# k2-fsa/Flow2GAN

Measured on AMD Instinct MI355X. Metric: audio-seconds/sec (train step, G+D fwd/bwd) mel_24k_base, higher is better.
Workload: dtype f32 (fp32-class products on the bf16 matrix pipe for the long reductions and the direct MRD convs: every fp32 operand as three bf16 pieces = 24 significand bits, the six v_mfma_f32_32x32x16_bf16 products with i + j <= 2 per fp32 product, fp32 accumulate, error <= 2^-23 per product; short reductions ; 1 GPU; mel_24k_base GAN stage-2 train step: D-step + G-step, each on its own batch (MPD+MRD+FM+multi-scale mel), fwd+bwd+grad all-reduce, no optimizer (metric is fwd/bwd); per_gpu_batch=64, gan=gan_multi_scale_mel_recon, parallelism=dp1, optimizer=none

## Files before the change

flow2gan_amd/csrc/conv32x6.hip:

```cpp
#include <stdlib.h>

#include "common.h"


namespace {

typedef float f32x16 __attribute__((ext_vector_type(16)));
typedef float f32x4 __attribute__((ext_vector_type(4)));
typedef __bf16 bf16x8 __attribute__((ext_vector_type(8)));
typedef unsigned int u32x2 __attribute__((ext_vector_type(2)));
typedef unsigned int u32x4 __attribute__((ext_vector_type(4)));

constexpr int C = 32, KH = 3, KW = 9, NTAP = KH * KW;
constexpr int PB = 208;
constexpr int TG = 4;
constexpr int WBB = C * PB;
constexpr int WCH = C * 12;

__device__ __attribute__((aligned(16))) float c6_zero[4] = {0.f, 0.f, 0.f, 0.f};

__device__ __forceinline__ void split3(const f32x4 v, u32x2& p0, u32x2& p1, u32x2& p2) {
  unsigned a0, a1, a2, b0, b1, b2;
  f2g_split3_pair(v.x, v.y, a0, a1, a2);
  f2g_split3_pair(v.z, v.w, b0, b1, b2);
  p0 = u32x2{a0, b0};
  p1 = u32x2{a1, b1};
  p2 = u32x2{a2, b2};
}

__device__ __forceinline__ void store_px3(unsigned char* p, const f32x4 v) {
  u32x2 p0, p1, p2;
  split3(v, p0, p1, p2);
// ... 31 lines not shown
  return (x * (D == 39 ? 1681 : D == 23 ? 2850 : D == 20 ? 3277 : 5462)) >> 16;
}

template <int TW_>
__device__ __forceinline__ void px_of_row(int pg, int r, int& ph, int& pw) {
  if (TW_ == 16) {
    ph = 2 * pg + (r >> 4);
    pw = (r + 12 * (r >> 4)) & 15;
  } else {
    const int p = pg * 32 + r;
    ph = p / TW_;
    pw = p % TW_;
  }
}

struct wplan {
  int src[3];
  int dst[3];
  int u[3];
};

template <int TH_, int TW_>
__global__ __launch_bounds__(512, 1) void conv32_s2_fwd6_kernel(const f2g_conv32_desc d, int tiles_w,
                                                               int tiles_h, int ntiles) {
  constexpr int IHv = TH_ + KH - 1, IWv = TW_ + (KW - 1) / 2, XW = 2 * IWv - 1;
  constexpr int SUBB = IHv * IWv * PB + 64;
  constexpr int NCHK = (IHv * XW * (C / 4) + 511) / 512;
  constexpr int NG = (NTAP + TG - 1) / TG + 1;
  static_assert(NG % 2 == 0, "the weight double buffer must come back to buffer 0 at a tile's end");
  static_assert(TH_ * TW_ == 128, "a block owns 128 output pixels");
  extern __shared__ __attribute__((aligned(16))) unsigned char smb[];
  unsigned char* At = smb;
  unsigned char* Bt = smb + 2 * SUBB;
  float* red = reinterpret_cast<float*>(Bt + 2 * TG * WBB);
  const int tid = threadIdx.x, lane = tid & 63, wave = tid >> 6;
  const int li = lane & 31, hh = lane >> 5;
  const int pg = wave & 3, half = wave >> 2;
  const int c4 = tid & 7;
  const int px0 = tid >> 3;
  auto tile_pos = [&](int tile, int& sq, int& h0, int& w0) {
    const int tw = tile % tiles_w, rest = tile / tiles_w;
    const int th = rest % tiles_h;
    sq = rest / tiles_h;
    h0 = th * TH_;
    w0 = tw * TW_;
  };
  auto load_patch = [&](int tile, f32x4 (&pf)[NCHK]) {
    int sq, h0, w0;
    tile_pos(tile, sq, h0, w0);
    const int x0 = 2 * w0 - (KW - 1) / 2;
    const float* org = d.x + (long long)sq * d.x_seq + (long long)(h0 - 1) * d.x_line + (long long)x0 * C + c4 * 4;
#pragma unroll
    for (int q = 0; q < NCHK; ++q) {
      const int px = px0 + 64 * q;
      const int r = div_small<XW>(px), xr = px - r * XW;
      const int h = h0 - 1 + r, x = x0 + xr;
      const bool ok = px < IHv * XW && h >= 0 && h < d.H && x >= 0 && x < d.Win;
      pf[q] = *reinterpret_cast<const f32x4*>(ok ? org + (long long)r * d.x_line + xr * C : c6_zero);
    }
  };
  auto store_patch = [&](const f32x4 (&pf)[NCHK]) {
#pragma unroll
    for (int q = 0; q < NCHK; ++q) {
      const int px = px0 + 64 * q;
      const int r = div_small<XW>(px), xr = px - r * XW;
      if (px < IHv * XW) store_px3(At + (xr & 1) * SUBB + (r * IWv + (xr >> 1)) * PB + c4 * 8, pf[q]);
    }
  };
  const unsigned char* wimg = reinterpret_cast<const unsigned char*>(d.w);
  wplan wp;
#pragma unroll
  for (int k = 0; k < 3; ++k) {
    const int c = tid + 512 * k;
    const int u = c / WCH, rem = c - u * WCH;
    const int row = rem / 12, part = rem - row * 12;
    wp.u[k] = u;
    wp.src[k] = row * (NTAP * 192) + part * 16;
    wp.dst[k] = u * WBB + row * PB + part * 16;
  }
  auto load_w = [&](int g, u32x4 (&wn)[3]) {
#pragma unroll
    for (int k = 0; k < 3; ++k) {
      int t = g * TG + wp.u[k];
      t = t < NTAP ? t : NTAP - 1;
      wn[k] = *reinterpret_cast<const u32x4*>(wimg + wp.src[k] + t * 192);
    }
  };
  auto store_w = [&](int buf, const u32x4 (&wn)[3]) {
#pragma unroll
    for (int k = 0; k < 3; ++k) *reinterpret_cast<u32x4*>(Bt + buf * (TG * WBB) + wp.dst[k]) = wn[k];
  };
  int ph, pw;
  px_of_row<TW_>(pg, li, ph, pw);
  const unsigned char* Ap = At + (ph * IWv + pw) * PB + hh * 16;
  const unsigned char* Bp = Bt + li * PB + hh * 16;
  const float bias = d.bias ? d.bias[li] : 0.f;

  int tile = blockIdx.x;
  if (tile >= ntiles) return;
  u32x4 wn[3];
  {
    f32x4 pf[NCHK];
    load_patch(tile, pf);
    load_w(0, wn);
    store_patch(pf);
    store_w(0, wn);
  }
  __syncthreads();
#define F2G_C6_AOFF(T) ((((T) % KW) & 1) * SUBB + (((T) / KW) * IWv + (((T) % KW) >> 1)) * PB)
  for (; tile < ntiles; tile += gridDim.x) {
    const int nxt = tile + gridDim.x;
    const bool more = nxt < ntiles;
    f32x4 pf[NCHK];
    load_patch(more ? nxt : tile, pf);
    f32x16 acc0, acc1;
#pragma unroll
    for (int e = 0; e < 16; ++e) { acc0[e] = 0.f; acc1[e] = 0.f; }
#pragma unroll
    for (int g = 0; g < NG; ++g) {
      load_w(g + 1 < NG ? g + 1 : 0, wn);
      const int buf = g & 1;
#pragma unroll
      for (int u2 = 0; u2 < 2; ++u2) {
        const int t0 = g * TG + u2, t1 = g * TG + 2 + u2;
        if (t0 < NTAP && (half ? t1 : t0) < NTAP)
          tap6(Ap + (half ? F2G_C6_AOFF(t1) : F2G_C6_AOFF(t0)), Bp + (buf * TG + half * 2 + u2) * WBB, acc0, acc1);
      }
      store_w(buf ^ 1, wn);
      __syncthreads();
    }
#undef F2G_C6_AOFF
#pragma unroll
    for (int e = 0; e < 16; ++e) acc0[e] += acc1[e];
    if (half == 1) {
#pragma unroll
      for (int e = 0; e < 16; ++e) red[(pg * 16 + e) * 64 + lane] = acc0[e];
    }
    if (more) store_patch(pf);
    __syncthreads();
    if (half == 0) {
      int sq, h0, w0;
      tile_pos(tile, sq, h0, w0);
      float* ys = d.y + (long long)sq * d.y_seq;
      float* turn = red + pg * (16 * 64);
      float v[16];
#pragma unroll
      for (int e = 0; e < 16; ++e) {
        v[e] = acc0[e] + red[(pg * 16 + e) * 64 + lane] + bias;
        if (d.lrelu_slope != 0.f) v[e] = v[e] > 0.f ? v[e] : d.lrelu_slope * v[e];
      }
      __builtin_amdgcn_wave_barrier();
#pragma unroll
      for (int e = 0; e < 16; ++e) turn[((e & 3) + 8 * (e >> 2) + 4 * hh) * 32 + li] = v[e];
      __builtin_amdgcn_wave_barrier();
#pragma unroll
      for (int j = 0; j < 4; ++j) {
        int qh, qw;
        px_of_row<TW_>(pg, (lane >> 3) + 8 * j, qh, qw);
        const int oh = h0 + qh, ow = w0 + qw;
        const f32x4 u = *reinterpret_cast<const f32x4*>(turn + ((lane >> 3) + 8 * j) * 32 + 4 * (lane & 7));
        if (oh < d.H && ow < d.Wout)
          *reinterpret_cast<f32x4*>(ys + (long long)oh * d.y_line + (long long)ow * C + 4 * (lane & 7)) = u;
      }
    }
  }
}

template <int TH_, int TW_>
__global__ __launch_bounds__(512, 1) void conv32_s2_dgrad6_kernel(const f2g_conv32_desc d, int tiles_w,
                                                                 int tiles_h, int ntiles) {
  constexpr int IHv = TH_ + KH - 1, GWv = TW_ + 4;
  constexpr int NCHK = (IHv * GWv * (C / 4) + 511) / 512;
  constexpr int NG = 8;
  static_assert(TH_ * TW_ == 128, "a block owns 128 positions of each column parity");
  extern __shared__ __attribute__((aligned(16))) unsigned char smb[];
  unsigned char* At = smb;
  unsigned char* Bt = smb + IHv * GWv * PB;
  float* turn = reinterpret_cast<float*>(Bt + 2 * TG * WBB) + (threadIdx.x >> 6) * (32 * 32);
  const int tid = threadIdx.x, lane = tid & 63, wave = tid >> 6;
  const int li = lane & 31, hh = lane >> 5;
  const int pg = wave & 3, E = wave >> 2;
  const int c4 = tid & 7;
  const int NU = E ? 4 : 5, NT = KH * NU;
  const int Wp = (d.Win + 1 - E) / 2;
  const int px0 = tid >> 3;
  auto tile_pos = [&](int tile, int& sq, int& h0, int& m0) {
    const int tw = tile % tiles_w, rest = tile / tiles_w;
    const int th = rest % tiles_h;
    sq = rest / tiles_h;
    h0 = th * TH_;
    m0 = tw * TW_;
  };
  auto load_patch = [&](int tile, f32x4 (&pf)[NCHK]) {
    int sq, h0, m0;
    tile_pos(tile, sq, h0, m0);
    const float* org = d.x + (long long)sq * d.x_seq + (long long)(h0 - 1) * d.x_line + (long long)(m0 - 2) * C + c4 * 4;
#pragma unroll
    for (int q = 0; q < NCHK; ++q) {
      const int px = px0 + 64 * q;
      const int r = div_small<GWv>(px), xc = px - r * GWv;
      const int h = h0 - 1 + r, c = m0 - 2 + xc;
      const bool ok = px < IHv * GWv && h >= 0 && h < d.H && c >= 0 && c < d.Wout;
      pf[q] = *reinterpret_cast<const f32x4*>(ok ? org + (long long)r * d.x_line + xc * C : c6_zero);
    }
  };
  auto store_patch = [&](const f32x4 (&pf)[NCHK]) {
#pragma unroll
    for (int q = 0; q < NCHK; ++q) {
      const int px = px0 + 64 * q;
      if (px < IHv * GWv) store_px3(At + px * PB + c4 * 8, pf[q]);
    }
  };
  const unsigned char* wimg = reinterpret_cast<const unsigned char*>(d.w);
  int wsrc[3], wdst[3], wslot[3];
#pragma unroll
  for (int k = 0; k < 3; ++k) {
    const int c = tid + 512 * k;
    const int u = c / WCH, rem = c - u * WCH;
    const int row = rem / 12, part = rem - row * 12;
    wslot[k] = u;
    wsrc[k] = row * 192 + part * 16;
    wdst[k] = u * WBB + row * PB + part * 16;
  }
  auto load_w = [&](int g, u32x4 (&wn)[3]) {
#pragma unroll
    for (int k = 0; k < 3; ++k) {
      const int e = wslot[k] >> 1, nu = e ? 4 : 5, nt = KH * nu;
      int ti = 2 * g + (wslot[k] & 1);
      ti = ti < nt ? ti : nt - 1;
      const int dh = e ? ti >> 2 : (ti * 13) >> 6;
      const int tile_w = dh * KW + e + 2 * (ti - dh * nu);
      wn[k] = *reinterpret_cast<const u32x4*>(wimg + (long long)tile_w * (C * 192) + wsrc[k]);
    }
  };
  auto store_w = [&](int buf, const u32x4 (&wn)[3]) {
#pragma unroll
    for (int k = 0; k < 3; ++k) *reinterpret_cast<u32x4*>(Bt + buf * (TG * WBB) + wdst[k]) = wn[k];
  };
  int ph, pw;
  px_of_row<TW_>(pg, li, ph, pw);
  const unsigned char* Ap = At + ((ph + 2) * GWv + pw + 4) * PB + hh * 16;
  const unsigned char* Bp = Bt + (E * 2) * WBB + li * PB + hh * 16;
  const bool msk = d.mask_src != nullptr, fm = d.fm_ref != nullptr;
  const float fmw = fm ? d.fm_w * (d.fm_wdev ? d.fm_wdev[0] : 1.f) : 0.f;
  float cs[4] = {0.f, 0.f, 0.f, 0.f};

  int tile = blockIdx.x;
  if (tile >= ntiles) return;
  u32x4 wn[3];
  {
    f32x4 pf[NCHK];
    load_patch(tile, pf);
    load_w(0, wn);
    store_patch(pf);
    store_w(0, wn);
  }
  __syncthreads();
  for (; tile < ntiles; tile += gridDim.x) {
    const int nxt = tile + gridDim.x;
    const bool more = nxt < ntiles;
    f32x4 pf[NCHK];
    load_patch(more ? nxt : tile, pf);
    int sq, h0, m0;
    tile_pos(tile, sq, h0, m0);
    long long ioff[4];
    f32x4 my[4];
#pragma unroll
    for (int j = 0; j < 4; ++j) {
      int qh, qw;
      px_of_row<TW_>(pg, (lane >> 3) + 8 * j, qh, qw);
      const int oh = h0 + qh, om = m0 + qw;
      ioff[j] = (oh < d.H && om < Wp)
                    ? (long long)sq * d.y_seq + (long long)oh * d.y_line + (long long)(2 * om + E) * C + 4 * (lane & 7)
                    : -1;
      if (msk && !fm) my[j] = *reinterpret_cast<const f32x4*>(d.mask_src + (ioff[j] >= 0 ? ioff[j] : 0));
    }
    f32x16 acc0, acc1;
#pragma unroll
    for (int e = 0; e < 16; ++e) { acc0[e] = 0.f; acc1[e] = 0.f; }
#define F2G_C6_GOFF(TI) ((E ? ((TI) / 4) * GWv + (TI) % 4 : ((TI) / 5) * GWv + (TI) % 5) * PB)
#pragma unroll
    for (int g = 0; g < NG; ++g) {
      load_w(g + 1 < NG ? g + 1 : 0, wn);
      const int buf = g & 1;
#pragma unroll
      for (int u2 = 0; u2 < 2; ++u2)
        if (2 * g + u2 < NT) tap6(Ap - F2G_C6_GOFF(2 * g + u2), Bp + (buf * TG + u2) * WBB, acc0, acc1);
      store_w(buf ^ 1, wn);
      __syncthreads();
    }
#undef F2G_C6_GOFF
#pragma unroll
    for (int q = 0; q < 16; ++q) turn[((q & 3) + 8 * (q >> 2) + 4 * hh) * 32 + li] = acc0[q] + acc1[q];
    __builtin_amdgcn_wave_barrier();
    auto item = [&](int j) {
      return *reinterpret_cast<const f32x4*>(turn + ((lane >> 3) + 8 * j) * 32 + 4 * (lane & 7));
    };
    if (!msk) {
#pragma unroll
      for (int j = 0; j < 4; ++j) {
        const f32x4 u = item(j);
        if (ioff[j] < 0) continue;
        cs[0] += u.x, cs[1] += u.y, cs[2] += u.z, cs[3] += u.w;
        *reinterpret_cast<f32x4*>(d.y + ioff[j]) = u;
      }
    } else if (!fm) {
#pragma unroll
      for (int j = 0; j < 4; ++j) {
        const f32x4 u = item(j);
        if (ioff[j] < 0) continue;
        f32x4 v;
        v.x = u.x * (my[j].x > 0.f ? 1.f : d.mask_slope);
        v.y = u.y * (my[j].y > 0.f ? 1.f : d.mask_slope);
        v.z = u.z * (my[j].z > 0.f ? 1.f : d.mask_slope);
        v.w = u.w * (my[j].w > 0.f ? 1.f : d.mask_slope);
        cs[0] += v.x, cs[1] += v.y, cs[2] += v.z, cs[3] += v.w;
        *reinterpret_cast<f32x4*>(d.y + ioff[j]) = v;
      }
    } else {
      f32x4 yv[4], fv[4];
#pragma unroll
      for (int j = 0; j < 4; ++j) {
        const long long o = ioff[j] >= 0 ? ioff[j] : 0;
        yv[j] = *reinterpret_cast<const f32x4*>(d.mask_src + o);
        fv[j] = *reinterpret_cast<const f32x4*>(d.fm_ref + o);
      }
#pragma unroll
      for (int j = 0; j < 4; ++j) {
        const f32x4 u = item(j);
        if (ioff[j] < 0) continue;
        float v[4] = {u.x, u.y, u.z, u.w};
        const float y[4] = {yv[j].x, yv[j].y, yv[j].z, yv[j].w}, f[4] = {fv[j].x, fv[j].y, fv[j].z, fv[j].w};
#pragma unroll
        for (int e = 0; e < 4; ++e) {
          const float dl = y[e] - f[e];
          v[e] += fmw * (dl > 0.f ? 1.f : (dl < 0.f ? -1.f : 0.f));
          v[e] *= y[e] > 0.f ? 1.f : d.mask_slope;
          cs[e] += v[e];
        }
        *reinterpret_cast<f32x4*>(d.y + ioff[j]) = f32x4{v[0], v[1], v[2], v[3]};
      }
    }
    __builtin_amdgcn_wave_barrier();
    if (more) store_patch(pf);
    __syncthreads();
  }
  if (d.colsum) {
#pragma unroll
    for (int e = 0; e < 4; ++e) {
      float v = cs[e];
      v += __shfl_xor(v, 8);
      v += __shfl_xor(v, 16);
      v += __shfl_xor(v, 32);
      if (lane < 8) atomicAdd(d.colsum + 4 * lane + e, v);
    }
  }
}

template <int TH_, int TW_>
__global__ __launch_bounds__(512, 1) void conv32_s2_dgrad6m_kernel(const f2g_conv32_desc d, int tiles_w,
                                                                 int tiles_h, int ntiles) {
  constexpr int IHv = TH_ + KH - 1, GWv = TW_ + 4;
  constexpr int NCHK = (IHv * GWv * (C / 4) + 511) / 512;
  constexpr int NG = 8;
  static_assert(TH_ * TW_ == 128, "a block owns 128 positions of each column parity");
  extern __shared__ __attribute__((aligned(16))) unsigned char smb[];
  unsigned char* At = smb;
  unsigned char* Bt = smb + IHv * GWv * PB;
  const int tid = threadIdx.x, lane = tid & 63, wave = tid >> 6;
  const int li = lane & 31, hh = lane >> 5;
  const int pg = wave & 3, E = wave >> 2;
  const int c4 = tid & 7;
  const int NU = E ? 4 : 5, NT = KH * NU;
  const int Wp = (d.Win + 1 - E) / 2;
  const int px0 = tid >> 3;
  auto tile_pos = [&](int tile, int& sq, int& h0, int& m0) {
    const int tw = tile % tiles_w, rest = tile / tiles_w;
    const int th = rest % tiles_h;
    sq = rest / tiles_h;
    h0 = th * TH_;
    m0 = tw * TW_;
  };
  auto load_patch = [&](int tile, f32x4 (&pf)[NCHK]) {
    int sq, h0, m0;
    tile_pos(tile, sq, h0, m0);
    const float* org = d.x + (long long)sq * d.x_seq + (long long)(h0 - 1) * d.x_line + (long long)(m0 - 2) * C + c4 * 4;
#pragma unroll
    for (int q = 0; q < NCHK; ++q) {
      const int px = px0 + 64 * q;
      const int r = div_small<GWv>(px), xc = px - r * GWv;
      const int h = h0 - 1 + r, c = m0 - 2 + xc;
      const bool ok = px < IHv * GWv && h >= 0 && h < d.H && c >= 0 && c < d.Wout;
      pf[q] = *reinterpret_cast<const f32x4*>(ok ? org + (long long)r * d.x_line + xc * C : c6_zero);
    }
  };
  auto store_patch = [&](const f32x4 (&pf)[NCHK]) {
#pragma unroll
    for (int q = 0; q < NCHK; ++q) {
      const int px = px0 + 64 * q;
      if (px < IHv * GWv) store_px3(At + px * PB + c4 * 8, pf[q]);
    }
  };
  const unsigned char* wimg = reinterpret_cast<const unsigned char*>(d.w);
  int wsrc[3], wdst[3], wslot[3];
#pragma unroll
  for (int k = 0; k < 3; ++k) {
    const int c = tid + 512 * k;
    const int u = c / WCH, rem = c - u * WCH;
    const int row = rem / 12, part = rem - row * 12;
    wslot[k] = u;
    wsrc[k] = row * 192 + part * 16;
    wdst[k] = u * WBB + row * PB + part * 16;
  }
  auto load_w = [&](int g, u32x4 (&wn)[3]) {
#pragma unroll
    for (int k = 0; k < 3; ++k) {
      const int e = wslot[k] >> 1, nu = e ? 4 : 5, nt = KH * nu;
      int ti = 2 * g + (wslot[k] & 1);
      ti = ti < nt ? ti : nt - 1;
      const int dh = e ? ti >> 2 : (ti * 13) >> 6;
      const int tile_w = dh * KW + e + 2 * (ti - dh * nu);
      wn[k] = *reinterpret_cast<const u32x4*>(wimg + (long long)tile_w * (C * 192) + wsrc[k]);
    }
  };
  auto store_w = [&](int buf, const u32x4 (&wn)[3]) {
#pragma unroll
    for (int k = 0; k < 3; ++k) *reinterpret_cast<u32x4*>(Bt + buf * (TG * WBB) + wdst[k]) = wn[k];
  };
  int ph, pw;
  px_of_row<TW_>(pg, li, ph, pw);
  const unsigned char* Ap = At + ((ph + 2) * GWv + pw + 4) * PB + hh * 16;
  const unsigned char* Bp = Bt + (E * 2) * WBB + li * PB + hh * 16;
  const bool msk = d.mask_src != nullptr, fm = d.fm_ref != nullptr;
  const float fmw = fm ? d.fm_w * (d.fm_wdev ? d.fm_wdev[0] : 1.f) : 0.f;
  float cs = 0.f;

  int tile = blockIdx.x;
  if (tile >= ntiles) return;
  u32x4 wn[3];
  {
    f32x4 pf[NCHK];
    load_patch(tile, pf);
    load_w(0, wn);
    store_patch(pf);
    store_w(0, wn);
  }
  __syncthreads();
  for (; tile < ntiles; tile += gridDim.x) {
    const int nxt = tile + gridDim.x;
    const bool more = nxt < ntiles;
    f32x4 pf[NCHK];
    load_patch(more ? nxt : tile, pf);
    int sq, h0, m0;
    tile_pos(tile, sq, h0, m0);
    float my[16];
    if (msk && !fm) {
#pragma unroll
      for (int q = 0; q < 16; ++q) {
        int qh, qw;
        px_of_row<TW_>(pg, (q & 3) + 8 * (q >> 2) + 4 * hh, qh, qw);
        const int oh = h0 + qh, om = m0 + qw;
        const long long off = (long long)sq * d.y_seq + (long long)oh * d.y_line + (long long)(2 * om + E) * C + li;
        my[q] = (oh < d.H && om < Wp) ? d.mask_src[off] : 1.f;
      }
    }
    f32x16 acc0, acc1;
#pragma unroll
    for (int e = 0; e < 16; ++e) { acc0[e] = 0.f; acc1[e] = 0.f; }
#define F2G_C6_GOFF(TI) ((E ? ((TI) / 4) * GWv + (TI) % 4 : ((TI) / 5) * GWv + (TI) % 5) * PB)
#pragma unroll
    for (int g = 0; g < NG; ++g) {
      load_w(g + 1 < NG ? g + 1 : 0, wn);
      const int buf = g & 1;
#pragma unroll
      for (int u2 = 0; u2 < 2; ++u2)
        if (2 * g + u2 < NT) tap6(Ap - F2G_C6_GOFF(2 * g + u2), Bp + (buf * TG + u2) * WBB, acc0, acc1);
      store_w(buf ^ 1, wn);
      __syncthreads();
    }
#undef F2G_C6_GOFF
#pragma unroll
    for (int q = 0; q < 16; ++q) {
      int qh, qw;
      px_of_row<TW_>(pg, (q & 3) + 8 * (q >> 2) + 4 * hh, qh, qw);
      const int oh = h0 + qh, om = m0 + qw;
      if (oh < d.H && om < Wp) {
        const long long off = (long long)sq * d.y_seq + (long long)oh * d.y_line + (long long)(2 * om + E) * C + li;
        float v = acc0[q] + acc1[q];
        if (msk) {
          const float y = fm ? d.mask_src[off] : my[q];
          if (fm) {
            const float dl = y - d.fm_ref[off];
            v += fmw * (dl > 0.f ? 1.f : (dl < 0.f ? -1.f : 0.f));
          }
          v *= y > 0.f ? 1.f : d.mask_slope;
        }
        cs += v;
        d.y[off] = v;
      }
    }
    if (more) store_patch(pf);
    __syncthreads();
  }
  if (d.colsum) {
    cs += __shfl_xor(cs, 32);
    if (hh == 0) atomicAdd(d.colsum + li, cs);
  }
}

typedef short s16x4 __attribute__((ext_vector_type(4)));
constexpr int GPL = 128 * 64;
constexpr int GCH = 128 * (C / 4) / 512;

__device__ __forceinline__ bf16x8 tr_pix8(const unsigned char* p) {
  typedef s16x4 __attribute__((address_space(3))) * lds_p;
  const s16x4 a = __builtin_amdgcn_ds_read_tr16_b64_v4i16((lds_p)(p));
  const s16x4 b = __builtin_amdgcn_ds_read_tr16_b64_v4i16((lds_p)(p + 4 * 64));
  return __builtin_bit_cast(bf16x8, __builtin_shufflevector(a, b, 0, 1, 2, 3, 4, 5, 6, 7));
}

template <int TH, int TW>
// ... 395 lines not shown
    if (wave == (t & 7)) {
#pragma unroll
      for (int e = 0; e < 16; ++e) {
        float v = 0.f;
#pragma unroll
        for (int w8 = 0; w8 < 8; ++w8) v += red[(w8 * 16 + e) * 64 + lane];
        const int co = (e & 3) + 8 * (e >> 2) + 4 * hh;
        atomicAdd(gw + co * (T33 * C) + t * C + li, v);
      }
    }
  }
}

template <int TH_, int TW_>
constexpr size_t fwd6_smem() {
  return (size_t)2 * ((TH_ + 2) * (TW_ + 4) * PB + 64) + 2 * TG * WBB + 4 * 16 * 64 * sizeof(float);
}
template <int TH_, int TW_>
constexpr size_t dgrad6_smem() {
  return (size_t)(TH_ + 2) * (TW_ + 4) * PB + 2 * TG * WBB + 8 * 32 * 32 * sizeof(float);
}

}

int f2g_conv32_fwd6_launch(const f2g_conv32_desc* d, hipStream_t st) {
  auto waste = [&](int th, int tw) {
    return (long long)((d->H + th - 1) / th * th) * ((d->Wout + tw - 1) / tw * tw);
  };
  const bool tall = waste(16, 8) < waste(8, 16);
  const int th = tall ? 16 : 8, tw = tall ? 8 : 16;
  const int tiles_h = (d->H + th - 1) / th, tiles_w = (d->Wout + tw - 1) / tw;
  const long long nt = (long long)tiles_h * tiles_w * d->S;
  if (nt >= (1ll << 30) || d->x_line >= (1ll << 24)) return F2G_EINVAL;
  static bool attr = false;
  if (!attr) {
// ... 10 lines not shown
  else
    hipLaunchKernelGGL((conv32_s2_fwd6_kernel<8, 16>), dim3(grid), dim3(512), (fwd6_smem<8, 16>()), st, *d,
                       tiles_w, tiles_h, (int)nt);
  return f2g_check_launch();
}

int f2g_conv32_dgrad6_launch(const f2g_conv32_desc* d, hipStream_t st) {
  const int Wp0 = (d->Win + 1) / 2;
  auto waste = [&](int th, int tw) {
    return (long long)((d->H + th - 1) / th * th) * ((Wp0 + tw - 1) / tw * tw);
  };
  const bool tall = waste(16, 8) < waste(8, 16);
  const int th = tall ? 16 : 8, tw = tall ? 8 : 16;
  const int tiles_h = (d->H + th - 1) / th, tiles_w = (Wp0 + tw - 1) / tw;
  const long long nt = (long long)tiles_h * tiles_w * d->S;
  if (nt >= (1ll << 30) || d->x_line >= (1ll << 24)) return F2G_EINVAL;
  static bool attr = false;
  if (!attr) {
    (void)hipFuncSetAttribute(reinterpret_cast<const void*>(conv32_s2_dgrad6_kernel<8, 16>),
                              hipFuncAttributeMaxDynamicSharedMemorySize, (int)(dgrad6_smem<8, 16>()));
    (void)hipFuncSetAttribute(reinterpret_cast<const void*>(conv32_s2_dgrad6_kernel<16, 8>),
                              hipFuncAttributeMaxDynamicSharedMemorySize, (int)(dgrad6_smem<16, 8>()));
    attr = true;
  }
  const int grid = (int)(nt < 256 ? nt : 256);
  if (d->mask_src) {
    static bool attrm = false;
    if (!attrm) {
      (void)hipFuncSetAttribute(reinterpret_cast<const void*>(conv32_s2_dgrad6m_kernel<8, 16>),
                                hipFuncAttributeMaxDynamicSharedMemorySize, (int)(dgrad6_smem<8, 16>()));
      (void)hipFuncSetAttribute(reinterpret_cast<const void*>(conv32_s2_dgrad6m_kernel<16, 8>),
                                hipFuncAttributeMaxDynamicSharedMemorySize, (int)(dgrad6_smem<16, 8>()));
      attrm = true;
    }
    if (tall)
      hipLaunchKernelGGL((conv32_s2_dgrad6m_kernel<16, 8>), dim3(grid), dim3(512), (dgrad6_smem<16, 8>()), st, *d,
                         tiles_w, tiles_h, (int)nt);
    else
      hipLaunchKernelGGL((conv32_s2_dgrad6m_kernel<8, 16>), dim3(grid), dim3(512), (dgrad6_smem<8, 16>()), st, *d,
                         tiles_w, tiles_h, (int)nt);
    return f2g_check_launch();
  }
  if (tall)
    hipLaunchKernelGGL((conv32_s2_dgrad6_kernel<16, 8>), dim3(grid), dim3(512), (dgrad6_smem<16, 8>()), st, *d,
                       tiles_w, tiles_h, (int)nt);
  else
    hipLaunchKernelGGL((conv32_s2_dgrad6_kernel<8, 16>), dim3(grid), dim3(512), (dgrad6_smem<8, 16>()), st, *d,
                       tiles_w, tiles_h, (int)nt);
  return f2g_check_launch();
}

int f2g_conv32_wgrad6_launch(const f2g_conv32_desc* d, float* gw, hipStream_t st) {
  auto waste = [&](int th, int tw) {
    return (long long)((d->H + th - 1) / th * th) * ((d->Wout + tw - 1) / tw * tw);
  };
  const bool tall = waste(16, 8) < waste(8, 16);
  const int th = tall ? 16 : 8, tw = tall ? 8 : 16;
// ... 88 lines not shown
```

Baseline: 793.2 audio-s/s.

## Keep conv32 weights in registers and split the reduction across waves

The stride-2 32-channel fwd and dgrad conv kernels stop staging weight taps through a double-buffered LDS ring with a barrier per tap group. Each wave now preloads its slice of the K reduction (tap halves) as bf16 split fragments in registers. It then sweeps all four pixel groups of the tile, and partial sums are reduced across the eight waves through LDS. This removes per-group weight loads, LDS stores and barriers, and it drops the separate masked dgrad kernel in favour of the unified one. The cost is much higher register pressure and a heavier cross-wave LDS reduction in the epilogue.

```diff
diff --git a/flow2gan_amd/csrc/conv32x6.hip b/flow2gan_amd/csrc/conv32x6.hip
--- a/flow2gan_amd/csrc/conv32x6.hip
+++ b/flow2gan_amd/csrc/conv32x6.hip
@@ -13,9 +13,6 @@
 
 constexpr int C = 32, KH = 3, KW = 9, NTAP = KH * KW;
 constexpr int PB = 208;
-constexpr int TG = 4;
-constexpr int WBB = C * PB;
-constexpr int WCH = C * 12;
 
 __device__ __attribute__((aligned(16))) float c6_zero[4] = {0.f, 0.f, 0.f, 0.f};
 
@@ -77,28 +74,22 @@
   }
 }
 
-struct wplan {
-  int src[3];
-  int dst[3];
-  int u[3];
-};
-
 template <int TH_, int TW_>
 __global__ __launch_bounds__(512, 1) void conv32_s2_fwd6_kernel(const f2g_conv32_desc d, int tiles_w,
                                                                int tiles_h, int ntiles) {
   constexpr int IHv = TH_ + KH - 1, IWv = TW_ + (KW - 1) / 2, XW = 2 * IWv - 1;
   constexpr int SUBB = IHv * IWv * PB + 64;
   constexpr int NCHK = (IHv * XW * (C / 4) + 511) / 512;
-  constexpr int NG = (NTAP + TG - 1) / TG + 1;
-  static_assert(NG % 2 == 0, "the weight double buffer must come back to buffer 0 at a tile's end");
+  constexpr int PGB = (TW_ == 16 ? 2 : 4) * IWv * PB;
+  constexpr int NKS = 2 * NTAP, KPW = 7;
   static_assert(TH_ * TW_ == 128, "a block owns 128 output pixels");
+  static_assert(6 * KPW + 2 * (KPW - 1) == NKS, "the k split covers the reduction exactly");
   extern __shared__ __attribute__((aligned(16))) unsigned char smb[];
   unsigned char* At = smb;
-  unsigned char* Bt = smb + 2 * SUBB;
-  float* red = reinterpret_cast<float*>(Bt + 2 * TG * WBB);
-  const int tid = threadIdx.x, lane = tid & 63, wave = tid >> 6;
+  float* red = reinterpret_cast<float*>(smb + 2 * SUBB);
+  const int tid = threadIdx.x, lane = tid & 63;
+  const int wave = __builtin_amdgcn_readfirstlane(tid >> 6);
   const int li = lane & 31, hh = lane >> 5;
-  const int pg = wave & 3, half = wave >> 2;
   const int c4 = tid & 7;
   const int px0 = tid >> 3;
   auto tile_pos = [&](int tile, int& sq, int& h0, int& w0) {
@@ -113,118 +104,117 @@
     tile_pos(tile, sq, h0, w0);
     const int x0 = 2 * w0 - (KW - 1) / 2;
     const float* org = d.x + (long long)sq * d.x_seq + (long long)(h0 - 1) * d.x_line + (long long)x0 * C + c4 * 4;
+    const int xl = (int)d.x_line;
+    int pxb = px0;
+    asm volatile("" : "+v"(pxb));
 #pragma unroll
     for (int q = 0; q < NCHK; ++q) {
-      const int px = px0 + 64 * q;
+      const int px = pxb + 64 * q;
       const int r = div_small<XW>(px), xr = px - r * XW;
       const int h = h0 - 1 + r, x = x0 + xr;
       const bool ok = px < IHv * XW && h >= 0 && h < d.H && x >= 0 && x < d.Win;
-      pf[q] = *reinterpret_cast<const f32x4*>(ok ? org + (long long)r * d.x_line + xr * C : c6_zero);
+      pf[q] = *reinterpret_cast<const f32x4*>(ok ? org + (r * xl + xr * C) : c6_zero);
     }
   };
   auto store_patch = [&](const f32x4 (&pf)[NCHK]) {
+    int pxb = px0;
+    asm volatile("" : "+v"(pxb));
 #pragma unroll
     for (int q = 0; q < NCHK; ++q) {
-      const int px = px0 + 64 * q;
+      const int px = pxb + 64 * q;
       const int r = div_small<XW>(px), xr = px - r * XW;
       if (px < IHv * XW) store_px3(At + (xr & 1) * SUBB + (r * IWv + (xr >> 1)) * PB + c4 * 8, pf[q]);
     }
   };
-  const unsigned char* wimg = reinterpret_cast<const unsigned char*>(d.w);
-  wplan wp;
-#pragma unroll
-  for (int k = 0; k < 3; ++k) {
-    const int c = tid + 512 * k;
-    const int u = c / WCH, rem = c - u * WCH;
-    const int row = rem / 12, part = rem - row * 12;
-    wp.u[k] = u;
-    wp.src[k] = row * (NTAP * 192) + part * 16;
-    wp.dst[k] = u * WBB + row * PB + part * 16;
-  }
-  auto load_w = [&](int g, u32x4 (&wn)[3]) {
-#pragma unroll
-    for (int k = 0; k < 3; ++k) {
-      int t = g * TG + wp.u[k];
-      t = t < NTAP ? t : NTAP - 1;
-      wn[k] = *reinterpret_cast<const u32x4*>(wimg + wp.src[k] + t * 192);
-    }
-  };
-  auto store_w = [&](int buf, const u32x4 (&wn)[3]) {
-#pragma unroll
-    for (int k = 0; k < 3; ++k) *reinterpret_cast<u32x4*>(Bt + buf * (TG * WBB) + wp.dst[k]) = wn[k];
-  };
-  int ph, pw;
-  px_of_row<TW_>(pg, li, ph, pw);
-  const unsigned char* Ap = At + (ph * IWv + pw) * PB + hh * 16;
-  const unsigned char* Bp = Bt + li * PB + hh * 16;
-  const float bias = d.bias ? d.bias[li] : 0.f;
-
   int tile = blockIdx.x;
   if (tile >= ntiles) return;
-  u32x4 wn[3];
+  f32x4 pf[NCHK];
+  load_patch(tile, pf);
+  const int k0 = wave * KPW - (wave == 7 ? 1 : 0);
+  const bool seven = wave < 6;
+  bf16x8 wf[KPW][3];
+  int koff[KPW];
   {
-    f32x4 pf[NCHK];
-    load_patch(tile, pf);
-    load_w(0, wn);
-    store_patch(pf);
-    store_w(0, wn);
-  }
+    const unsigned char* wrow = reinterpret_cast<const unsigned char*>(d.w) + li * (NTAP * 192) + hh * 16;
+#pragma unroll
+    for (int j = 0; j < KPW; ++j) {
+      int k = k0 + j;
+      k = k < NKS ? k : NKS - 1;
+      const int t = k >> 1, ks = k & 1;
+      const int dh = t / KW, jw = t - dh * KW;
+      koff[j] = (jw & 1) * SUBB + (dh * IWv + (jw >> 1)) * PB + ks * 32;
+#pragma unroll
+      for (int q = 0; q < 3; ++q) wf[j][q] = *reinterpret_cast<const bf16x8*>(wrow + t * 192 + q * 64 + ks * 32);
+    }
+  }
+  int ph, pw;
+  px_of_row<TW_>(0, li, ph, pw);
+  const unsigned char* Ap = At + (ph * IWv + pw) * PB + hh * 16;
+  const int orow = (wave & 3) * 8 + (lane >> 3), och = 4 * (lane & 7);
+  f32x4 bias4 = {0.f, 0.f, 0.f, 0.f};
+  if (d.bias) bias4 = f32x4{d.bias[och], d.bias[och + 1], d.bias[och + 2], d.bias[och + 3]};
+  store_patch(pf);
   __syncthreads();
-#define F2G_C6_AOFF(T) ((((T) % KW) & 1) * SUBB + (((T) / KW) * IWv + (((T) % KW) >> 1)) * PB)
   for (; tile < ntiles; tile += gridDim.x) {
     const int nxt = tile + gridDim.x;
     const bool more = nxt < ntiles;
-    f32x4 pf[NCHK];
     load_patch(more ? nxt : tile, pf);
-    f32x16 acc0, acc1;
-#pragma unroll
-    for (int e = 0; e < 16; ++e) { acc0[e] = 0.f; acc1[e] = 0.f; }
-#pragma unroll
-    for (int g = 0; g < NG; ++g) {
-      load_w(g + 1 < NG ? g + 1 : 0, wn);
-      const int buf = g & 1;
-#pragma unroll
-      for (int u2 = 0; u2 < 2; ++u2) {
-        const int t0 = g * TG + u2, t1 = g * TG + 2 + u2;
-        if (t0 < NTAP && (half ? t1 : t0) < NTAP)
-          tap6(Ap + (half ? F2G_C6_AOFF(t1) : F2G_C6_AOFF(t0)), Bp + (buf * TG + half * 2 + u2) * WBB, acc0, acc1);
-      }
-      store_w(buf ^ 1, wn);
+    f32x16 acc[4];
+#pragma unroll
+    for (int g4 = 0; g4 < 4; ++g4)
+#pragma unroll
+      for (int e = 0; e < 16; ++e) acc[g4][e] = 0.f;
+    bf16x8 a[2][3];
+#pragma unroll
+    for (int q = 0; q < 3; ++q) a[0][q] = *reinterpret_cast<const bf16x8*>(Ap + koff[0] + q * 64);
+#pragma unroll
+    for (int u = 0; u < 4 * KPW; ++u) {
+      const int j = u >> 2, g4 = u & 3;
+      if (u + 1 < 4 * KPW) {
+        const unsigned char* an = Ap + koff[(u + 1) >> 2] + ((u + 1) & 3) * PGB;
+#pragma unroll
+        for (int q = 0; q < 3; ++q) a[(u + 1) & 1][q] = *reinterpret_cast<const bf16x8*>(an + q * 64);
+      }
+      __builtin_amdgcn_sched_barrier(0);
+      if (j < KPW - 1 || seven) {
+#define F2G_X6_ONE(I, J) acc[g4] = __builtin_amdgcn_mfma_f32_32x32x16_bf16(a[u & 1][I], wf[j][J], acc[g4], 0, 0, 0);
+        F2G_X6_ONE(2, 0) F2G_X6_ONE(1, 1) F2G_X6_ONE(0, 2) F2G_X6_ONE(1, 0) F2G_X6_ONE(0, 1) F2G_X6_ONE(0, 0)
+#undef F2G_X6_ONE
+      }
+      __builtin_amdgcn_sched_barrier(0);
+    }
+    int sq, h0, w0;
+    tile_pos(tile, sq, h0, w0);
+    float* ys = d.y + (long long)sq * d.y_seq;
+    __syncthreads();
+#pragma unroll
+    for (int p2 = 0; p2 < 2; ++p2) {
+      if (p2) __syncthreads();
+#pragma unroll
+      for (int g2 = 0; g2 < 2; ++g2)
+#pragma unroll
+        for (int e = 0; e < 16; ++e)
+          red[((wave * 2 + g2) * 32 + (e & 3) + 8 * (e >> 2) + 4 * hh) * 32 + li] = acc[2 * p2 + g2][e];
       __syncthreads();
-    }
-#undef F2G_C6_AOFF
-#pragma unroll
-    for (int e = 0; e < 16; ++e) acc0[e] += acc1[e];
-    if (half == 1) {
-#pragma unroll
-      for (int e = 0; e < 16; ++e) red[(pg * 16 + e) * 64 + lane] = acc0[e];
-    }
-    if (more) store_patch(pf);
-    __syncthreads();
-    if (half == 0) {
-      int sq, h0, w0;
-      tile_pos(tile, sq, h0, w0);
-      float* ys = d.y + (long long)sq * d.y_seq;
-      float* turn = red + pg * (16 * 64);
-      float v[16];
-#pragma unroll
-      for (int e = 0; e < 16; ++e) {
-        v[e] = acc0[e] + red[(pg * 16 + e) * 64 + lane] + bias;
-        if (d.lrelu_slope != 0.f) v[e] = v[e] > 0.f ? v[e] : d.lrelu_slope * v[e];
-      }
-      __builtin_amdgcn_wave_barrier();
-#pragma unroll
-      for (int e = 0; e < 16; ++e) turn[((e & 3) + 8 * (e >> 2) + 4 * hh) * 32 + li] = v[e];
-      __builtin_amdgcn_wave_barrier();
-#pragma unroll
-      for (int j = 0; j < 4; ++j) {
-        int qh, qw;
-        px_of_row<TW_>(pg, (lane >> 3) + 8 * j, qh, qw);
-        const int oh = h0 + qh, ow = w0 + qw;
-        const f32x4 u = *reinterpret_cast<const f32x4*>(turn + ((lane >> 3) + 8 * j) * 32 + 4 * (lane & 7));
-        if (oh < d.H && ow < d.Wout)
-          *reinterpret_cast<f32x4*>(ys + (long long)oh * d.y_line + (long long)ow * C + 4 * (lane & 7)) = u;
-      }
+      f32x4 s = *reinterpret_cast<const f32x4*>(red + (((wave >> 2)) * 32 + orow) * 32 + och);
+#pragma unroll
+      for (int w8 = 1; w8 < 8; ++w8) {
+        const f32x4 v = *reinterpret_cast<const f32x4*>(red + ((w8 * 2 + (wave >> 2)) * 32 + orow) * 32 + och);
+        s.x += v.x, s.y += v.y, s.z += v.z, s.w += v.w;
+      }
+      s.x += bias4.x, s.y += bias4.y, s.z += bias4.z, s.w += bias4.w;
+      if (d.lrelu_slope != 0.f) {
+        s.x = s.x > 0.f ? s.x : d.lrelu_slope * s.x;
+        s.y = s.y > 0.f ? s.y : d.lrelu_slope * s.y;
+        s.z = s.z > 0.f ? s.z : d.lrelu_slope * s.z;
+        s.w = s.w > 0.f ? s.w : d.lrelu_slope * s.w;
+      }
+      int qh, qw;
+      px_of_row<TW_>(2 * p2 + (wave >> 2), orow, qh, qw);
+      const int oh = h0 + qh, ow = w0 + qw;
+      if (oh < d.H && ow < d.Wout)
+        *reinterpret_cast<f32x4*>(ys + (long long)oh * d.y_line + (long long)ow * C + och) = s;
+      if (p2 == 0 && more) store_patch(pf);
     }
   }
 }
@@ -234,17 +224,18 @@
                                                                  int tiles_h, int ntiles) {
   constexpr int IHv = TH_ + KH - 1, GWv = TW_ + 4;
   constexpr int NCHK = (IHv * GWv * (C / 4) + 511) / 512;
-  constexpr int NG = 8;
+  constexpr int PGB = (TW_ == 16 ? 2 : 4) * GWv * PB;
+  constexpr int KPW = 8;
   static_assert(TH_ * TW_ == 128, "a block owns 128 positions of each column parity");
   extern __shared__ __attribute__((aligned(16))) unsigned char smb[];
   unsigned char* At = smb;
-  unsigned char* Bt = smb + IHv * GWv * PB;
-  float* turn = reinterpret_cast<float*>(Bt + 2 * TG * WBB) + (threadIdx.x >> 6) * (32 * 32);
-  const int tid = threadIdx.x, lane = tid & 63, wave = tid >> 6;
+  float* red = reinterpret_cast<float*>(smb + IHv * GWv * PB);
+  const int tid = threadIdx.x, lane = tid & 63;
+  const int wave = __builtin_amdgcn_readfirstlane(tid >> 6);
   const int li = lane & 31, hh = lane >> 5;
-  const int pg = wave & 3, E = wave >> 2;
+  const int wq = wave & 3, E = wave >> 2;
   const int c4 = tid & 7;
-  const int NU = E ? 4 : 5, NT = KH * NU;
+  const int NU = E ? 4 : 5;
   const int Wp = (d.Win + 1 - E) / 2;
   const int px0 = tid >> 3;
   auto tile_pos = [&](int tile, int& sq, int& h0, int& m0) {
@@ -258,13 +249,16 @@
     int sq, h0, m0;
     tile_pos(tile, sq, h0, m0);
     const float* org = d.x + (long long)sq * d.x_seq + (long long)(h0 - 1) * d.x_line + (long long)(m0 - 2) * C + c4 * 4;
+    const int xl = (int)d.x_line;
+    int pxb = px0;
+    asm volatile("" : "+v"(pxb));
 #pragma unroll
     for (int q = 0; q < NCHK; ++q) {
-      const int px = px0 + 64 * q;
+      const int px = pxb + 64 * q;
       const int r = div_small<GWv>(px), xc = px - r * GWv;
       const int h = h0 - 1 + r, c = m0 - 2 + xc;
       const bool ok = px < IHv * GWv && h >= 0 && h < d.H && c >= 0 && c < d.Wout;
-      pf[q] = *reinterpret_cast<const f32x4*>(ok ? org + (long long)r * d.x_line + xc * C : c6_zero);
+      pf[q] = *reinterpret_cast<const f32x4*>(ok ? org + (r * xl + xc * C) : c6_zero);
     }
   };
   auto store_patch = [&](const f32x4 (&pf)[NCHK]) {
@@ -274,300 +268,155 @@
       if (px < IHv * GWv) store_px3(At + px * PB + c4 * 8, pf[q]);
     }
   };
-  const unsigned char* wimg = reinterpret_cast<const unsigned char*>(d.w);
-  int wsrc[3], wdst[3], wslot[3];
-#pragma unroll
-  for (int k = 0; k < 3; ++k) {
-    const int c = tid + 512 * k;
-    const int u = c / WCH, rem = c - u * WCH;
-    const int row = rem / 12, part = rem - row * 12;
-    wslot[k] = u;
-    wsrc[k] = row * 192 + part * 16;
-    wdst[k] = u * WBB + row * PB + part * 16;
-  }
-  auto load_w = [&](int g, u32x4 (&wn)[3]) {
-#pragma unroll
-    for (int k = 0; k < 3; ++k) {
-      const int e = wslot[k] >> 1, nu = e ? 4 : 5, nt = KH * nu;
-      int ti = 2 * g + (wslot[k] & 1);
-      ti = ti < nt ? ti : nt - 1;
-      const int dh = e ? ti >> 2 : (ti * 13) >> 6;
-      const int tile_w = dh * KW + e + 2 * (ti - dh * nu);
-      wn[k] = *reinterpret_cast<const u32x4*>(wimg + (long long)tile_w * (C * 192) + wsrc[k]);
-    }
-  };
-  auto store_w = [&](int buf, const u32x4 (&wn)[3]) {
-#pragma unroll
-    for (int k = 0; k < 3; ++k) *reinterpret_cast<u32x4*>(Bt + buf * (TG * WBB) + wdst[k]) = wn[k];
-  };
+  int tile = blockIdx.x;
+  if (tile >= ntiles) return;
+  f32x4 pf[NCHK];
+  load_patch(tile, pf);
+  const int nk = E ? 6 : (wq < 2 ? 8 : 7);
+  const int k0 = E ? 6 * wq : (wq < 2 ? 8 * wq : 16 + 7 * (wq - 2));
+  bf16x8 wf[KPW][3];
+  int koff[KPW];
+  {
+    const unsigned char* wrow = reinterpret_cast<const unsigned char*>(d.w) + li * 192 + hh * 16;
+    const int nks = 2 * KH * NU;
+#pragma unroll
+    for (int j = 0; j < KPW; ++j) {
+      int k = k0 + j;
+      k = k < nks ? k : nks - 1;
+      const int ti = k >> 1, ks = k & 1;
+      const int dh = E ? ti >> 2 : (ti * 13) >> 6;
+      const int u = ti - dh * NU;
+      koff[j] = ks * 32 - (dh * GWv + u) * PB;
+      const int tile_w = dh * KW + E + 2 * u;
+#pragma unroll
+      for (int q = 0; q < 3; ++q)
+        wf[j][q] = *reinterpret_cast<const bf16x8*>(wrow + tile_w * (C * 192) + q * 64 + ks * 32);
+    }
+  }
   int ph, pw;
-  px_of_row<TW_>(pg, li, ph, pw);
+  px_of_row<TW_>(0, li, ph, pw);
   const unsigned char* Ap = At + ((ph + 2) * GWv + pw + 4) * PB + hh * 16;
-  const unsigned char* Bp = Bt + (E * 2) * WBB + li * PB + hh * 16;
+  const int och = 4 * (lane & 7);
   const bool msk = d.mask_src != nullptr, fm = d.fm_ref != nullptr;
   const float fmw = fm ? d.fm_w * (d.fm_wdev ? d.fm_wdev[0] : 1.f) : 0.f;
   float cs[4] = {0.f, 0.f, 0.f, 0.f};
-
-  int tile = blockIdx.x;
-  if (tile >= ntiles) return;
-  u32x4 wn[3];
-  {
-    f32x4 pf[NCHK];
-    load_patch(tile, pf);
-    load_w(0, wn);
-    store_patch(pf);
-    store_w(0, wn);
-  }
+  store_patch(pf);
   __syncthreads();
   for (; tile < ntiles; tile += gridDim.x) {
     const int nxt = tile + gridDim.x;
     const bool more = nxt < ntiles;
-    f32x4 pf[NCHK];
     load_patch(more ? nxt : tile, pf);
     int sq, h0, m0;
     tile_pos(tile, sq, h0, m0);
-    long long ioff[4];
+    const long long tbase = (long long)sq * d.y_seq + (long long)h0 * d.y_line + (long long)(2 * m0 + E) * C;
+    auto item_off = [&](int jj) {
+      int qh, qw, l8 = lane >> 3;
+      asm volatile("" : "+v"(l8));
+      px_of_row<TW_>(2 * (jj >> 1) + (wq >> 1), (wq & 1) * 16 + l8 + 8 * (jj & 1), qh, qw);
+      return (h0 + qh < d.H && m0 + qw < Wp) ? qh * (int)d.y_line + 2 * qw * C + och : -1;
+    };
     f32x4 my[4];
-#pragma unroll
-    for (int j = 0; j < 4; ++j) {
-      int qh, qw;
-      px_of_row<TW_>(pg, (lane >> 3) + 8 * j, qh, qw);
-      const int oh = h0 + qh, om = m0 + qw;
-      ioff[j] = (oh < d.H && om < Wp)
-                    ? (long long)sq * d.y_seq + (long long)oh * d.y_line + (long long)(2 * om + E) * C + 4 * (lane & 7)
-                    : -1;
-      if (msk && !fm) my[j] = *reinterpret_cast<const f32x4*>(d.mask_src + (ioff[j] >= 0 ? ioff[j] : 0));
-    }
-    f32x16 acc0, acc1;
-#pragma unroll
-    for (int e = 0; e < 16; ++e) { acc0[e] = 0.f; acc1[e] = 0.f; }
-#define F2G_C6_GOFF(TI) ((E ? ((TI) / 4) * GWv + (TI) % 4 : ((TI) / 5) * GWv + (TI) % 5) * PB)
-#pragma unroll
-    for (int g = 0; g < NG; ++g) {
-      load_w(g + 1 < NG ? g + 1 : 0, wn);
-      const int buf = g & 1;
-#pragma unroll
-      for (int u2 = 0; u2 < 2; ++u2)
-        if (2 * g + u2 < NT) tap6(Ap - F2G_C6_GOFF(2 * g + u2), Bp + (buf * TG + u2) * WBB, acc0, acc1);
-      store_w(buf ^ 1, wn);
+    if (msk && !fm) {
+#pragma unroll
+      for (int jj = 0; jj < 4; ++jj) {
+        const int o = item_off(jj);
+        my[jj] = *reinterpret_cast<const f32x4*>(d.mask_src + (o >= 0 ? tbase + o : 0));
+      }
+    }
+    f32x16 acc[4];
+#pragma unroll
+    for (int g4 = 0; g4 < 4; ++g4)
+#pragma unroll
+      for (int e = 0; e < 16; ++e) acc[g4][e] = 0.f;
+    bf16x8 a[2][3];
+#pragma unroll
+    for (int q = 0; q < 3; ++q) a[0][q] = *reinterpret_cast<const bf16x8*>(Ap + koff[0] + q * 64);
+#pragma unroll
+    for (int u = 0; u < 4 * KPW; ++u) {
+      const int j = u >> 2, g4 = u & 3;
+      if (u + 1 < 4 * KPW) {
+        const unsigned char* an = Ap + koff[(u + 1) >> 2] + ((u + 1) & 3) * PGB;
+#pragma unroll
+        for (int q = 0; q < 3; ++q) a[(u + 1) & 1][q] = *reinterpret_cast<const bf16x8*>(an + q * 64);
+      }
+      __builtin_amdgcn_sched_barrier(0);
+      if (j < 6 || j < nk) {
+#define F2G_X6_ONE(I, J) acc[g4] = __builtin_amdgcn_mfma_f32_32x32x16_bf16(a[u & 1][I], wf[j][J], acc[g4], 0, 0, 0);
+        F2G_X6_ONE(2, 0) F2G_X6_ONE(1, 1) F2G_X6_ONE(0, 2) F2G_X6_ONE(1, 0) F2G_X6_ONE(0, 1) F2G_X6_ONE(0, 0)
+#undef F2G_X6_ONE
+      }
+      __builtin_amdgcn_sched_barrier(0);
+    }
+    __syncthreads();
+#pragma unroll
+    for (int p2 = 0; p2 < 2; ++p2) {
+      if (p2) __syncthreads();
+      f32x4 fv[2];
+      if (msk && fm) {
+#pragma unroll
+        for (int i2 = 0; i2 < 2; ++i2) {
+          const int o = item_off(2 * p2 + i2);
+          const long long oo = o >= 0 ? tbase + o : 0;
+          my[2 * p2 + i2] = *reinterpret_cast<const f32x4*>(d.mask_src + oo);
+          fv[i2] = *reinterpret_cast<const f32x4*>(d.fm_ref + oo);
+        }
+      }
+#pragma unroll
+      for (int g2 = 0; g2 < 2; ++g2)
+#pragma unroll
+        for (int e = 0; e < 16; ++e)
+          red[((wave * 2 + g2) * 32 + (e & 3) + 8 * (e >> 2) + 4 * hh) * 32 + li] = acc[2 * p2 + g2][e];
       __syncthreads();
-    }
-#undef F2G_C6_GOFF
-#pragma unroll
-    for (int q = 0; q < 16; ++q) turn[((q & 3) + 8 * (q >> 2) + 4 * hh) * 32 + li] = acc0[q] + acc1[q];
-    __builtin_amdgcn_wave_barrier();
-    auto item = [&](int j) {
-      return *reinterpret_cast<const f32x4*>(turn + ((lane >> 3) + 8 * j) * 32 + 4 * (lane & 7));
-    };
-    if (!msk) {
-#pragma unroll
-      for (int j = 0; j < 4; ++j) {
-        const f32x4 u = item(j);
-        if (ioff[j] < 0) continue;
-        cs[0] += u.x, cs[1] += u.y, cs[2] += u.z, cs[3] += u.w;
-        *reinterpret_cast<f32x4*>(d.y + ioff[j]) = u;
-      }
-    } else if (!fm) {
-#pragma unroll
-      for (int j = 0; j < 4; ++j) {
-        const f32x4 u = item(j);
-        if (ioff[j] < 0) continue;
-        f32x4 v;
-        v.x = u.x * (my[j].x > 0.f ? 1.f : d.mask_slope);
-        v.y = u.y * (my[j].y > 0.f ? 1.f : d.mask_slope);
-        v.z = u.z * (my[j].z > 0.f ? 1.f : d.mask_slope);
-        v.w = u.w * (my[j].w > 0.f ? 1.f : d.mask_slope);
-        cs[0] += v.x, cs[1] += v.y, cs[2] += v.z, cs[3] += v.w;
-        *reinterpret_cast<f32x4*>(d.y + ioff[j]) = v;
-      }
-    } else {
-      f32x4 yv[4], fv[4];
-#pragma unroll
-      for (int j = 0; j < 4; ++j) {
-        const long long o = ioff[j] >= 0 ? ioff[j] : 0;
-        yv[j] = *reinterpret_cast<const f32x4*>(d.mask_src + o);
-        fv[j] = *reinterpret_cast<const f32x4*>(d.fm_ref + o);
-      }
-#pragma unroll
-      for (int j = 0; j < 4; ++j) {
-        const f32x4 u = item(j);
-        if (ioff[j] < 0) continue;
-        float v[4] = {u.x, u.y, u.z, u.w};
-        const float y[4] = {yv[j].x, yv[j].y, yv[j].z, yv[j].w}, f[4] = {fv[j].x, fv[j].y, fv[j].z, fv[j].w};
-#pragma unroll
-        for (int e = 0; e < 4; ++e) {
-          const float dl = y[e] - f[e];
-          v[e] += fmw * (dl > 0.f ? 1.f : (dl < 0.f ? -1.f : 0.f));
-          v[e] *= y[e] > 0.f ? 1.f : d.mask_slope;
-          cs[e] += v[e];
+#pragma unroll
+      for (int i2 = 0; i2 < 2; ++i2) {
+        const int jj = 2 * p2 + i2;
+        const float* rp = red + (((E * 4) * 2 + (wq >> 1)) * 32 + (wq & 1) * 16 + (lane >> 3) + 8 * i2) * 32 + och;
+        f32x4 s = *reinterpret_cast<const f32x4*>(rp);
+#pragma unroll
+        for (int w4 = 1; w4 < 4; ++w4) {
+          const f32x4 v = *reinterpret_cast<const f32x4*>(rp + w4 * (2 * 32 * 32));
+          s.x += v.x, s.y += v.y, s.z += v.z, s.w += v.w;
         }
-        *reinterpret_cast<f32x4*>(d.y + ioff[j]) = f32x4{v[0], v[1], v[2], v[3]};
-      }
-    }
-    __builtin_amdgcn_wave_barrier();
-    if (more) store_patch(pf);
-    __syncthreads();
+        const int o = item_off(jj);
+        if (o < 0) continue;
+        float v[4] = {s.x, s.y, s.z, s.w};
+        if (msk && !fm) {
+          const float y[4] = {my[jj].x, my[jj].y, my[jj].z, my[jj].w};
+#pragma unroll
+          for (int e = 0; e < 4; ++e) v[e] *= y[e] > 0.f ? 1.f : d.mask_slope;
+        } else if (msk) {
+          const float y[4] = {my[jj].x, my[jj].y, my[jj].z, my[jj].w}, f[4] = {fv[i2].x, fv[i2].y, fv[i2].z, fv[i2].w};
+#pragma unroll
+          for (int e = 0; e < 4; ++e) {
+            const float dl = y[e] - f[e];
+            v[e] += fmw * (dl > 0.f ? 1.f : (dl < 0.f ? -1.f : 0.f));
+            v[e] *= y[e] > 0.f ? 1.f : d.mask_slope;
+          }
+        }
+#pragma unroll
+        for (int e = 0; e < 4; ++e) cs[e] += v[e];
+        *reinterpret_cast<f32x4*>(d.y + tbase + o) = f32x4{v[0], v[1], v[2], v[3]};
+      }
+      if (p2 == 0 && more) store_patch(pf);
+    }
   }
   if (d.colsum) {
+    float* csl = reinterpret_cast<float*>(At);
 #pragma unroll
     for (int e = 0; e < 4; ++e) {
       float v = cs[e];
       v += __shfl_xor(v, 8);
       v += __shfl_xor(v, 16);
       v += __shfl_xor(v, 32);
-      if (lane < 8) atomicAdd(d.colsum + 4 * lane + e, v);
-    }
-  }
-}
-
-template <int TH_, int TW_>
-__global__ __launch_bounds__(512, 1) void conv32_s2_dgrad6m_kernel(const f2g_conv32_desc d, int tiles_w,
-                                                                 int tiles_h, int ntiles) {
-  constexpr int IHv = TH_ + KH - 1, GWv = TW_ + 4;
-  constexpr int NCHK = (IHv * GWv * (C / 4) + 511) / 512;
-  constexpr int NG = 8;
-  static_assert(TH_ * TW_ == 128, "a block owns 128 positions of each column parity");
-  extern __shared__ __attribute__((aligned(16))) unsigned char smb[];
-  unsigned char* At = smb;
-  unsigned char* Bt = smb + IHv * GWv * PB;
-  const int tid = threadIdx.x, lane = tid & 63, wave = tid >> 6;
-  const int li = lane & 31, hh = lane >> 5;
-  const int pg = wave & 3, E = wave >> 2;
-  const int c4 = tid & 7;
-  const int NU = E ? 4 : 5, NT = KH * NU;
-  const int Wp = (d.Win + 1 - E) / 2;
-  const int px0 = tid >> 3;
-  auto tile_pos = [&](int tile, int& sq, int& h0, int& m0) {
-    const int tw = tile % tiles_w, rest = tile / tiles_w;
-    const int th = rest % tiles_h;
-    sq = rest / tiles_h;
-    h0 = th * TH_;
-    m0 = tw * TW_;
-  };
-  auto load_patch = [&](int tile, f32x4 (&pf)[NCHK]) {
-    int sq, h0, m0;
-    tile_pos(tile, sq, h0, m0);
-    const float* org = d.x + (long long)sq * d.x_seq + (long long)(h0 - 1) * d.x_line + (long long)(m0 - 2) * C + c4 * 4;
-#pragma unroll
-    for (int q = 0; q < NCHK; ++q) {
-      const int px = px0 + 64 * q;
-      const int r = div_small<GWv>(px), xc = px - r * GWv;
-      const int h = h0 - 1 + r, c = m0 - 2 + xc;
-      const bool ok = px < IHv * GWv && h >= 0 && h < d.H && c >= 0 && c < d.Wout;
-      pf[q] = *reinterpret_cast<const f32x4*>(ok ? org + (long long)r * d.x_line + xc * C : c6_zero);
-    }
-  };
-  auto store_patch = [&](const f32x4 (&pf)[NCHK]) {
-#pragma unroll
-    for (int q = 0; q < NCHK; ++q) {
-      const int px = px0 + 64 * q;
-      if (px < IHv * GWv) store_px3(At + px * PB + c4 * 8, pf[q]);
-    }
-  };
-  const unsigned char* wimg = reinterpret_cast<const unsigned char*>(d.w);
-  int wsrc[3], wdst[3], wslot[3];
-#pragma unroll
-  for (int k = 0; k < 3; ++k) {
-    const int c = tid + 512 * k;
-    const int u = c / WCH, rem = c - u * WCH;
-    const int row = rem / 12, part = rem - row * 12;
-    wslot[k] = u;
-    wsrc[k] = row * 192 + part * 16;
-    wdst[k] = u * WBB + row * PB + part * 16;
-  }
-  auto load_w = [&](int g, u32x4 (&wn)[3]) {
-#pragma unroll
-    for (int k = 0; k < 3; ++k) {
-      const int e = wslot[k] >> 1, nu = e ? 4 : 5, nt = KH * nu;
-      int ti = 2 * g + (wslot[k] & 1);
-      ti = ti < nt ? ti : nt - 1;
-      const int dh = e ? ti >> 2 : (ti * 13) >> 6;
-      const int tile_w = dh * KW + e + 2 * (ti - dh * nu);
-      wn[k] = *reinterpret_cast<const u32x4*>(wimg + (long long)tile_w * (C * 192) + wsrc[k]);
-    }
-  };
-  auto store_w = [&](int buf, const u32x4 (&wn)[3]) {
-#pragma unroll
-    for (int k = 0; k < 3; ++k) *reinterpret_cast<u32x4*>(Bt + buf * (TG * WBB) + wdst[k]) = wn[k];
-  };
-  int ph, pw;
-  px_of_row<TW_>(pg, li, ph, pw);
-  const unsigned char* Ap = At + ((ph + 2) * GWv + pw + 4) * PB + hh * 16;
-  const unsigned char* Bp = Bt + (E * 2) * WBB + li * PB + hh * 16;
-  const bool msk = d.mask_src != nullptr, fm = d.fm_ref != nullptr;
-  const float fmw = fm ? d.fm_w * (d.fm_wdev ? d.fm_wdev[0] : 1.f) : 0.f;
-  float cs = 0.f;
-
-  int tile = blockIdx.x;
-  if (tile >= ntiles) return;
-  u32x4 wn[3];
-  {
-    f32x4 pf[NCHK];
-    load_patch(tile, pf);
-    load_w(0, wn);
-    store_patch(pf);
-    store_w(0, wn);
-  }
-  __syncthreads();
-  for (; tile < ntiles; tile += gridDim.x) {
-    const int nxt = tile + gridDim.x;
-    const bool more = nxt < ntiles;
-    f32x4 pf[NCHK];
-    load_patch(more ? nxt : tile, pf);
-    int sq, h0, m0;
-    tile_pos(tile, sq, h0, m0);
-    float my[16];
-    if (msk && !fm) {
-#pragma unroll
-      for (int q = 0; q < 16; ++q) {
-        int qh, qw;
-        px_of_row<TW_>(pg, (q & 3) + 8 * (q >> 2) + 4 * hh, qh, qw);
-        const int oh = h0 + qh, om = m0 + qw;
-        const long long off = (long long)sq * d.y_seq + (long long)oh * d.y_line + (long long)(2 * om + E) * C + li;
-        my[q] = (oh < d.H && om < Wp) ? d.mask_src[off] : 1.f;
-      }
-    }
-    f32x16 acc0, acc1;
-#pragma unroll
-    for (int e = 0; e < 16; ++e) { acc0[e] = 0.f; acc1[e] = 0.f; }
-#define F2G_C6_GOFF(TI) ((E ? ((TI) / 4) * GWv + (TI) % 4 : ((TI) / 5) * GWv + (TI) % 5) * PB)
-#pragma unroll
-    for (int g = 0; g < NG; ++g) {
-      load_w(g + 1 < NG ? g + 1 : 0, wn);
-      const int buf = g & 1;
-#pragma unroll
-      for (int u2 = 0; u2 < 2; ++u2)
-        if (2 * g + u2 < NT) tap6(Ap - F2G_C6_GOFF(2 * g + u2), Bp + (buf * TG + u2) * WBB, acc0, acc1);
-      store_w(buf ^ 1, wn);
-      __syncthreads();
-    }
-#undef F2G_C6_GOFF
-#pragma unroll
-    for (int q = 0; q < 16; ++q) {
-      int qh, qw;
-      px_of_row<TW_>(pg, (q & 3) + 8 * (q >> 2) + 4 * hh, qh, qw);
-      const int oh = h0 + qh, om = m0 + qw;
-      if (oh < d.H && om < Wp) {
-        const long long off = (long long)sq * d.y_seq + (long long)oh * d.y_line + (long long)(2 * om + E) * C + li;
-        float v = acc0[q] + acc1[q];
-        if (msk) {
-          const float y = fm ? d.mask_src[off] : my[q];
-          if (fm) {
-            const float dl = y - d.fm_ref[off];
-            v += fmw * (dl > 0.f ? 1.f : (dl < 0.f ? -1.f : 0.f));
-          }
-          v *= y > 0.f ? 1.f : d.mask_slope;
-        }
-        cs += v;
-        d.y[off] = v;
-      }
-    }
-    if (more) store_patch(pf);
-    __syncthreads();
-  }
-  if (d.colsum) {
-    cs += __shfl_xor(cs, 32);
-    if (hh == 0) atomicAdd(d.colsum + li, cs);
+      if (lane < 8) csl[wave * 32 + 4 * lane + e] = v;
+    }
+    __syncthreads();
+    if (tid < 32) {
+      float v = csl[tid];
+#pragma unroll
+      for (int w8 = 1; w8 < 8; ++w8) v += csl[w8 * 32 + tid];
+      atomicAdd(d.colsum + tid, v);
+    }
   }
 }
 
@@ -993,11 +842,11 @@
 
 template <int TH_, int TW_>
 constexpr size_t fwd6_smem() {
-  return (size_t)2 * ((TH_ + 2) * (TW_ + 4) * PB + 64) + 2 * TG * WBB + 4 * 16 * 64 * sizeof(float);
+  return (size_t)2 * ((TH_ + 2) * (TW_ + 4) * PB + 64) + 8 * 2 * 32 * 32 * sizeof(float);
 }
 template <int TH_, int TW_>
 constexpr size_t dgrad6_smem() {
-  return (size_t)(TH_ + 2) * (TW_ + 4) * PB + 2 * TG * WBB + 8 * 32 * 32 * sizeof(float);
+  return (size_t)(TH_ + 2) * (TW_ + 4) * PB + 8 * 2 * 32 * 32 * sizeof(float);
 }
 
 }
@@ -1038,7 +887,7 @@
   const int th = tall ? 16 : 8, tw = tall ? 8 : 16;
   const int tiles_h = (d->H + th - 1) / th, tiles_w = (Wp0 + tw - 1) / tw;
   const long long nt = (long long)tiles_h * tiles_w * d->S;
-  if (nt >= (1ll << 30) || d->x_line >= (1ll << 24)) return F2G_EINVAL;
+  if (nt >= (1ll << 30) || d->x_line >= (1ll << 24) || d->y_line >= (1ll << 24)) return F2G_EINVAL;
   static bool attr = false;
   if (!attr) {
     (void)hipFuncSetAttribute(reinterpret_cast<const void*>(conv32_s2_dgrad6_kernel<8, 16>),
@@ -1048,23 +897,6 @@
     attr = true;
   }
   const int grid = (int)(nt < 256 ? nt : 256);
-  if (d->mask_src) {
-    static bool attrm = false;
-    if (!attrm) {
-      (void)hipFuncSetAttribute(reinterpret_cast<const void*>(conv32_s2_dgrad6m_kernel<8, 16>),
-                                hipFuncAttributeMaxDynamicSharedMemorySize, (int)(dgrad6_smem<8, 16>()));
-      (void)hipFuncSetAttribute(reinterpret_cast<const void*>(conv32_s2_dgrad6m_kernel<16, 8>),
-                                hipFuncAttributeMaxDynamicSharedMemorySize, (int)(dgrad6_smem<16, 8>()));
-      attrm = true;
-    }
-    if (tall)
-      hipLaunchKernelGGL((conv32_s2_dgrad6m_kernel<16, 8>), dim3(grid), dim3(512), (dgrad6_smem<16, 8>()), st, *d,
-                         tiles_w, tiles_h, (int)nt);
-    else
-      hipLaunchKernelGGL((conv32_s2_dgrad6m_kernel<8, 16>), dim3(grid), dim3(512), (dgrad6_smem<8, 16>()), st, *d,
-                         tiles_w, tiles_h, (int)nt);
-    return f2g_check_launch();
-  }
   if (tall)
     hipLaunchKernelGGL((conv32_s2_dgrad6_kernel<16, 8>), dim3(grid), dim3(512), (dgrad6_smem<16, 8>()), st, *d,
                        tiles_w, tiles_h, (int)nt);
```

New measurement: 805.4 audio-s/s, median of 6. 1.02x the previous value.
